# sidward14/gan-lab

Hardware: AMD Instinct MI355X
Metric: images/sec (G+D step), StyleGAN 1024^2 bs32/GPU (higher is better)
Workload: dtype f32; 1 GPU; StyleGAN res_samples=1024 FFHQ-shaped synthetic, bs=32/GPU fp32, nonsaturating + R1(lambda=10) + drift, stabilised phase, 1 D-iter + 1 G-iter; global_batch=32, per_gpu_batch=32, parallelism=single

## Files before the change

gan_lab_amd/csrc/pointwise.hip:

```cpp
#include "common.h"

#include <stdlib.h>

namespace {

constexpr int kMaxBlocks = 256 * 8;

inline unsigned ew_blocks(long long n_items) {
  long long b = (n_items + 255) / 256;
  if (b < 1) b = 1;
  if (b > kMaxBlocks) b = kMaxBlocks;
  return (unsigned)b;
}

struct ChunkRange { long long begin, end, stride; };
__device__ __forceinline__ ChunkRange chunk_range(long long hw4, int chunks, int c, int contig) {
  ChunkRange r;
  if (contig) {
    const long long rows = (hw4 + 255) / 256, per = (rows + chunks - 1) / chunks;
    r.begin = (long long)c * per * 256;
    r.end = r.begin + per * 256;
    if (r.end > hw4) r.end = hw4;
    r.stride = 256;
  } else {
// ... 298 lines not shown
  const double inv = 1.0 / (double)HW;
  const double k = rd * ys, a1 = (double)s1[pl] * inv, a2 = (double)s2[pl] * inv;
  const float* pg = gy + pl * HW;
  const float* px = x + pl * HW;
  const float* pn = (want_nw && noise) ? noise + (long long)n * HW : nullptr;
  float* po = out + pl * HW;
  const int lane = threadIdx.x & 63;
  double sb = 0.0, snw = 0.0;
  auto zval = [&](float g, float v) -> double {
    double t = k * ((double)g - a1 - ((double)v - md) * rd * a2);
    if (act == GANLAB_ACT_LRELU && !(v > 0.f)) t *= (double)slope;
    return t;
  };
  for (long long base = chunk * 256LL; base < per_n; base += (long long)chunks * 256) {
    const long long i = base + threadIdx.x;
    const bool live = i < per_n;
    const long long ii = live ? i : per_n - 1;
    const int rr = (int)(ii / w4), q = (int)(ii - (long long)rr * w4);
    const int y0 = R * rr, x0 = 4 * q;
    float h[R + 2][4];
#pragma unroll
    for (int kk = 0; kk < R + 2; ++kk) {
      const int yy = y0 - 1 + kk;
      const bool valid = (unsigned)yy < (unsigned)H;
      const long long ro = (long long)yy * W;
      float z[4] = {0.f, 0.f, 0.f, 0.f};
      if (valid) {
        float g[4], v[4];
        *reinterpret_cast<float4*>(g) = *reinterpret_cast<const float4*>(pg + ro + x0);
        *reinterpret_cast<float4*>(v) = *reinterpret_cast<const float4*>(px + ro + x0);
        const bool own = live && kk >= 1 && kk <= R;
        float nz[4] = {0.f, 0.f, 0.f, 0.f};
        if (own && pn) *reinterpret_cast<float4*>(nz) = *reinterpret_cast<const float4*>(pn + ro + x0);
#pragma unroll
        for (int j = 0; j < 4; ++j) {
          const double t = zval(g[j], v[j]);
          z[j] = (float)t;
          if (own) {
            sb += t;
            snw += t * (double)nz[j];
          }
        }
      }
      float l = __shfl_up(z[3], 1, 64);
      float r = __shfl_down(z[0], 1, 64);
      const bool need_l = lane == 0 && q != 0, need_r = lane == 63 && q != w4 - 1;
      float e = 0.f;
      if (valid && (need_l || need_r)) {
        const long long eo = ro + x0 + (need_l ? -1 : 4);
        e = (float)zval(pg[eo], px[eo]);
      }
      if (q == 0) l = 0.f;
      else if (lane == 0) l = e;
      if (q == w4 - 1) r = 0.f;
      else if (lane == 63) r = e;
      h[kk][0] = l + 2.f * z[0] + z[1];
      h[kk][1] = z[0] + 2.f * z[1] + z[2];
      h[kk][2] = z[1] + 2.f * z[2] + z[3];
      h[kk][3] = z[2] + 2.f * z[3] + r;
    }
    if (!live) continue;
#pragma unroll
    for (int kk = 0; kk < R; ++kk) {
      float4 o;
      o.x = (h[kk][0] + 2.f * h[kk + 1][0] + h[kk + 2][0]) * 0.0625f;
      o.y = (h[kk][1] + 2.f * h[kk + 1][1] + h[kk + 2][1]) * 0.0625f;
      o.z = (h[kk][2] + 2.f * h[kk + 1][2] + h[kk + 2][2]) * 0.0625f;
      o.w = (h[kk][3] + 2.f * h[kk + 1][3] + h[kk + 2][3]) * 0.0625f;
      *reinterpret_cast<float4*>(po + (long long)(y0 + kk) * W + x0) = o;
    }
  }
  const long long slot = ((long long)c * N + n) * chunks + chunk;
  if (want_b) {
    sb = gl_block_sum_256d(sb, red);
    if (threadIdx.x == 0) part[slot] = sb;
  }
  if (want_nw) {
    if (want_b) __syncthreads();
    snw = gl_block_sum_256d(snw, red);
    if (threadIdx.x == 0) part[(long long)C * N * chunks + slot] = snw;
  }
}

inline int blur_rows(int H) { return (H & 3) == 0 ? 4 : 2; }
inline int blur_rows_mode(int H, int mode) {
  const int min8 = mode == BF_FWD ? 512 : (mode == BF_A ? 256 : (1 << 30));
  return ((H & 7) == 0 && H >= min8) ? 8 : blur_rows(H);
}
#define BLUR_FUSED_LAUNCH(MODE, ...)                                                                   \
  do {                                                                                                 \
    const int rows_ = blur_rows_mode(H, MODE);                                                         \
    if (rows_ == 8) GL_LAUNCH((blur_fused_kernel<MODE, 8>), dim3(chunks, C), dim3(256), 0, ST, __VA_ARGS__);      \
    else if (rows_ == 4) GL_LAUNCH((blur_fused_kernel<MODE, 4>), dim3(chunks, C), dim3(256), 0, ST, __VA_ARGS__); \
    else GL_LAUNCH((blur_fused_kernel<MODE, 2>), dim3(chunks, C), dim3(256), 0, ST, __VA_ARGS__);                \
  } while (0)

#define BLUR_FUSED_LAUNCH_BITS(MODE, ...)                                                                            \
  do {                                                                                                               \
    const int rows_ = blur_rows_mode(H, MODE);                                                                       \
    if (rows_ == 8) GL_LAUNCH((blur_fused_kernel<MODE, 8, false, true>), dim3(chunks, C), dim3(256), 0, ST, __VA_ARGS__);      \
    else if (rows_ == 4) GL_LAUNCH((blur_fused_kernel<MODE, 4, false, true>), dim3(chunks, C), dim3(256), 0, ST, __VA_ARGS__); \
    else GL_LAUNCH((blur_fused_kernel<MODE, 2, false, true>), dim3(chunks, C), dim3(256), 0, ST, __VA_ARGS__);                \
  } while (0)

inline int blur_fused_chunks(int N, int H, int W) {
  long long c = ((long long)N * (H / blur_rows(H)) * (W / 4) + 256 * 4 - 1) / (256 * 4);
  if (c < 1) c = 1;
  if (c > 128) c = 128;
  return (int)c;
}

__global__ __launch_bounds__(256) void bias_act_stats_kernel(const float* __restrict__ x, const float* __restrict__ bias,
                                                             const float* __restrict__ noise,
                                                             const float* __restrict__ noise_w, float* __restrict__ y,
                                                             double* __restrict__ spart, int C, long long hw4,
                                                             int chunks, float bias_scale, int act, float slope,
                                                             int contig) {
  __shared__ double dred[2][4];
  const long long pl = blockIdx.y;
  const int c = (int)(pl % C);
  const long long n = pl / C;
  const float b = bias ? bias[c] * bias_scale : 0.f;
  const float nw = noise ? noise_w[c] : 0.f;
  const float4* xp = reinterpret_cast<const float4*>(x) + pl * hw4;
  const float4* np = noise ? reinterpret_cast<const float4*>(noise) + n * hw4 : nullptr;
  float4* yp = reinterpret_cast<float4*>(y) + pl * hw4;
  double ds = 0.0, dss = 0.0;
  const ChunkRange cr = chunk_range(hw4, chunks, blockIdx.x, contig);
  for (long long i = cr.begin + threadIdx.x; i < cr.end; i += cr.stride) {
    float v[4], nz[4] = {0.f, 0.f, 0.f, 0.f};
    *reinterpret_cast<float4*>(v) = xp[i];
    if (np) *reinterpret_cast<float4*>(nz) = np[i];
#pragma unroll
    for (int k = 0; k < 4; ++k) {
      float t = v[k] + b + nw * nz[k];
      if (act == GANLAB_ACT_LRELU) t = gl_lrelu(t, slope);
      v[k] = t;
      const double d = (double)t;
      ds += d;
      dss += d * d;
    }
    yp[i] = *reinterpret_cast<float4*>(v);
  }
#pragma unroll
  for (int o = 32; o > 0; o >>= 1) {
    ds += __shfl_xor(ds, o, 64);
    dss += __shfl_xor(dss, o, 64);
  }
  if ((threadIdx.x & 63) == 0) {
    dred[0][threadIdx.x >> 6] = ds;
    dred[1][threadIdx.x >> 6] = dss;
  }
  __syncthreads();
  if (threadIdx.x < 2) {
    const int k = threadIdx.x;
    spart[(pl * chunks + blockIdx.x) * 2 + k] = (dred[k][0] + dred[k][1]) + (dred[k][2] + dred[k][3]);
  }
}

__global__ void act_stats_finish_kernel(const double* __restrict__ spart, float* __restrict__ mean,
                                        float* __restrict__ rstd, long long planes, int chunks, double inv_hw, float eps) {
  const long long pl = blockIdx.x * (long long)blockDim.x + threadIdx.x;
  if (pl >= planes) return;
  double s = 0.0, ss = 0.0;
  for (int k = 0; k < chunks; ++k) {
    s += spart[(pl * chunks + k) * 2];
    ss += spart[(pl * chunks + k) * 2 + 1];
  }
  const double m = s * inv_hw;
  double var = ss * inv_hw - m * m;
  if (var < 0.0) var = 0.0;
  mean[pl] = (float)m;
  rstd[pl] = (float)(1.0 / sqrt(var + (double)eps));
}

__global__ __launch_bounds__(256) void row_stats_partial_kernel(const float* __restrict__ x, double* __restrict__ spart,
                                                                int chunks, long long m4) {
  __shared__ double red[2][4];
  const long long row = blockIdx.x / chunks;
  const int k = blockIdx.x % chunks;
  const long long per = (m4 + chunks - 1) / chunks, lo = k * per, hi = lo + per < m4 ? lo + per : m4;
  const float4* p4 = reinterpret_cast<const float4*>(x) + row * m4;
  double s = 0.0, ss = 0.0;
  for (long long i = lo + threadIdx.x; i < hi; i += 256) {
    const float4 v = p4[i];
    const double a = (double)v.x, b = (double)v.y, c = (double)v.z, d = (double)v.w;
    s += (a + b) + (c + d);
    ss += (a * a + b * b) + (c * c + d * d);
  }
#pragma unroll
  for (int o = 32; o > 0; o >>= 1) {
    s += __shfl_xor(s, o, 64);
    ss += __shfl_xor(ss, o, 64);
// ... 1158 lines not shown
  if (gb) GL_LAUNCH(channel_sum_stage2, dim3(C), dim3(64), 0, ST, (const double*)part, gb, C, N * chunks, bias_scale);
  if (gnw)
    GL_LAUNCH(channel_sum_stage2, dim3(C), dim3(64), 0, ST, (const double*)part + (size_t)C * N * chunks, gnw, C,
              N * chunks, 1.f);
  return GL_CHECK_LAUNCH();
}

int ganlab_instnorm_bwd_rgb_supported(int N, int C, int crgb, long long HW) {
  return (N > 0 && N <= 65535 && C > 0 && C <= 16 && crgb > 0 && crgb <= 4 && HW >= 1024 && (HW & 3) == 0) ? 1 : 0;
}

static RgbSrc make_rgb_src(const float* grgb, const float* wp, int crgb, int C) {
  RgbSrc r;
  r.grgb = grgb; r.wp = wp; r.crgb = crgb; r.cout_p = (C + 63) / 64 * 64;
  return r;
}

size_t ganlab_instnorm_bwd_reduce_rgb_workspace(int N, int C, long long HW) {
  if (!ganlab_instnorm_bwd_rgb_supported(N, C, 3, HW)) return 0;
  return (size_t)N * C * act_stats_chunks(HW / 4) * 2 * sizeof(double);
}

int ganlab_instnorm_style_bwd_reduce_rgb_f32(const float* grgb, const float* wp, int crgb, const float* x,
                                             const float* mean, const float* rstd, float* s1, float* s2, int N, int C,
                                             long long HW, void* workspace, size_t workspace_bytes, void* stream) {
  if (!grgb || !wp || !x || !mean || !rstd || !s1 || !s2) return GANLAB_EINVAL;
  if (!ganlab_instnorm_bwd_rgb_supported(N, C, crgb, HW)) return GANLAB_EUNSUPPORTED;
  if (!workspace || workspace_bytes < ganlab_instnorm_bwd_reduce_rgb_workspace(N, C, HW)) return GANLAB_EWORKSPACE;
  const long long hw4 = HW / 4, planes = (long long)N * C;
  const int chunks = act_stats_chunks(hw4);
  double* part = reinterpret_cast<double*>(workspace);
  if (C == RGB_MAXC && crgb == 3)
    GL_LAUNCH(instnorm_bwd_reduce_rgb_kernel<true>, dim3((unsigned)chunks, (unsigned)N), dim3(256), 0, ST,
              make_rgb_src(grgb, wp, crgb, C), x, mean, rstd, part, C, hw4, chunks, pw_contig());
  else
    GL_LAUNCH(instnorm_bwd_reduce_rgb_kernel<false>, dim3((unsigned)chunks, (unsigned)N), dim3(256), 0, ST,
              make_rgb_src(grgb, wp, crgb, C), x, mean, rstd, part, C, hw4, chunks, pw_contig());
  GL_LAUNCH(instnorm_bwd_reduce_rgb_finish_kernel, dim3((unsigned)((planes + 63) / 64)), dim3(64), 0, ST,
            (const double*)part, s1, s2, planes, chunks);
  return GL_CHECK_LAUNCH();
}

int ganlab_instnorm_style_bwd_act_rgb_f32(const float* grgb, const float* wp, int crgb, const float* x, const float* mean,
                                          const float* rstd, const float* style, const float* s1, const float* s2,
                                          const float* noise, float* gz, float* gb, float* gnw, int N, int C, long long HW,
                                          int act, float slope, float bias_scale, void* workspace, size_t workspace_bytes,
                                          void* stream) {
  if (!grgb || !wp || !x || !mean || !rstd || !s1 || !s2 || !gz || (gnw && !noise)) return GANLAB_EINVAL;
  if (!ganlab_instnorm_bwd_rgb_supported(N, C, crgb, HW)) return GANLAB_EUNSUPPORTED;
  if ((gb || gnw) && (!workspace || workspace_bytes < ganlab_instnorm_bwd_act_workspace(N, C, HW)))
    return GANLAB_EWORKSPACE;
  const long long hw4 = HW / 4;
  const int chunks = act_stats_chunks(hw4);
  double* part = reinterpret_cast<double*>(workspace);
  if (C == RGB_MAXC && crgb == 3 && act == GANLAB_ACT_LRELU)
    GL_LAUNCH(instnorm_bwd_apply_act_rgb_kernel<true>, dim3((unsigned)chunks, (unsigned)N), dim3(256), 0, ST,
              make_rgb_src(grgb, wp, crgb, C), x, mean, rstd, style, s1, s2, noise, gz, part, N, C, hw4, chunks, act, slope,
              gb ? 1 : 0, gnw ? 1 : 0, pw_contig());
  else
    GL_LAUNCH(instnorm_bwd_apply_act_rgb_kernel<false>, dim3((unsigned)chunks, (unsigned)N), dim3(256), 0, ST,
              make_rgb_src(grgb, wp, crgb, C), x, mean, rstd, style, s1, s2, noise, gz, part, N, C, hw4, chunks, act, slope,
              gb ? 1 : 0, gnw ? 1 : 0, pw_contig());
  if (gb) GL_LAUNCH(channel_sum_stage2, dim3(C), dim3(64), 0, ST, (const double*)part, gb, C, N * chunks, bias_scale);
  if (gnw)
    GL_LAUNCH(channel_sum_stage2, dim3(C), dim3(64), 0, ST, (const double*)part + (size_t)C * N * chunks, gnw, C,
              N * chunks, 1.f);
  return GL_CHECK_LAUNCH();
}

int ganlab_instnorm_style_bwd_act_blur_f32(const float* gy, const float* x, const float* mean, const float* rstd,
                                           const float* style, const float* s1, const float* s2, const float* noise,
                                           float* out, float* gb, float* gnw, int N, int C, int H, int W, int act,
                                           float slope, float bias_scale, void* workspace, size_t workspace_bytes,
                                           void* stream) {
  if (!gy || !x || !mean || !rstd || !s1 || !s2 || !out || N <= 0 || C <= 0 || (gnw && !noise)) return GANLAB_EINVAL;
  if (!ganlab_blur_fused_supported(H, W) || N > 65535 || C > 65535) return GANLAB_EUNSUPPORTED;
  const long long HW = (long long)H * W;
  if ((gb || gnw) && (!workspace || workspace_bytes < ganlab_instnorm_bwd_act_workspace(N, C, HW))) return GANLAB_EWORKSPACE;
  const int rows = blur_rows(H);
  const long long per_n = (long long)(H / rows) * (W / 4);
  int chunks = (int)((per_n + 256 * 4 - 1) / (256 * 4));
  if (chunks < 1) chunks = 1;
  if (chunks > 64) chunks = 64;
  double* part = reinterpret_cast<double*>(workspace);
  const dim3 grid((unsigned)chunks, (unsigned)C, (unsigned)N);
  if (rows == 4)
    GL_LAUNCH(instnorm_bwd_act_blur_kernel<4>, grid, dim3(256), 0, ST, gy, x, mean, rstd, style, s1, s2, noise, out, part, N, C,
              H, W, chunks, act, slope, gb ? 1 : 0, gnw ? 1 : 0);
  else
    GL_LAUNCH(instnorm_bwd_act_blur_kernel<2>, grid, dim3(256), 0, ST, gy, x, mean, rstd, style, s1, s2, noise, out, part, N, C,
              H, W, chunks, act, slope, gb ? 1 : 0, gnw ? 1 : 0);
  if (gb) GL_LAUNCH(channel_sum_stage2, dim3(C), dim3(64), 0, ST, (const double*)part, gb, C, N * chunks, bias_scale);
  if (gnw)
    GL_LAUNCH(channel_sum_stage2, dim3(C), dim3(64), 0, ST, (const double*)part + (size_t)C * N * chunks, gnw, C,
              N * chunks, 1.f);
  return GL_CHECK_LAUNCH();
}

int ganlab_bias_act_stats_f32(const float* x, const float* bias, const float* noise, const float* noise_w, float* y,
                              float* mean, float* rstd, int N, int C, long long HW, float bias_scale, int act,
                              float slope, float eps, void* workspace, size_t workspace_bytes, void* stream) {
  if (!x || !y || !mean || !rstd || N <= 0 || C <= 0 || HW <= 0 || (noise && !noise_w)) return GANLAB_EINVAL;
  if ((HW & 3) != 0) return GANLAB_EUNSUPPORTED;
  if (!workspace || workspace_bytes < ganlab_act_stats_workspace(N, C, HW)) return GANLAB_EWORKSPACE;
  const long long hw4 = HW / 4, planes = (long long)N * C;
  const int chunks = act_stats_chunks(hw4);
  double* sp = reinterpret_cast<double*>(workspace);
  GL_LAUNCH(bias_act_stats_kernel, dim3((unsigned)chunks, (unsigned)planes), dim3(256), 0, ST, x, bias, noise, noise_w,
            y, sp, C, hw4, chunks, bias_scale, act, slope, pw_contig());
  GL_LAUNCH(act_stats_finish_kernel, dim3((unsigned)((planes + 255) / 256)), dim3(256), 0, ST, (const double*)sp, mean,
            rstd, planes, chunks, 1.0 / (double)HW, eps);
  return GL_CHECK_LAUNCH();
}

int ganlab_blur_bias_act_stats_f32(const float* x, const float* bias, const float* noise, const float* noise_w,
                                   float* y, float* mean, float* rstd, int N, int C, int H, int W, float bias_scale,
                                   int act, float slope, float eps, void* workspace, size_t workspace_bytes,
                                   void* stream) {
  if (!x || !y || !mean || !rstd || N <= 0 || C <= 0 || (noise && !noise_w)) return GANLAB_EINVAL;
  if (!ganlab_blur_fused_supported(H, W)) return GANLAB_EUNSUPPORTED;
  if (!workspace || workspace_bytes < ganlab_act_stats_workspace(N, C, (long long)H * W)) return GANLAB_EWORKSPACE;
  const int rows = blur_rows_mode(H, BF_FWD);
  long long per_n = (long long)(H / rows) * (W / 4);
  int chunks = (int)((per_n + 256 * 4 - 1) / (256 * 4));
  if (chunks < 1) chunks = 1;
  if (chunks > 128) chunks = 128;
  double* sp = reinterpret_cast<double*>(workspace);
  const dim3 grid((unsigned)chunks, (unsigned)C, (unsigned)N);
  if (rows == 8)
    GL_LAUNCH((blur_fused_kernel<BF_FWD, 8, true>), grid, dim3(256), 0, ST, x, (const float*)nullptr, noise, bias,
              noise_w, y, (double*)nullptr, N, C, H, W, chunks, bias_scale, act, slope, 0, sp);
  else if (rows == 4)
    GL_LAUNCH((blur_fused_kernel<BF_FWD, 4, true>), grid, dim3(256), 0, ST, x, (const float*)nullptr, noise, bias,
              noise_w, y, (double*)nullptr, N, C, H, W, chunks, bias_scale, act, slope, 0, sp);
  else
    GL_LAUNCH((blur_fused_kernel<BF_FWD, 2, true>), grid, dim3(256), 0, ST, x, (const float*)nullptr, noise, bias,
              noise_w, y, (double*)nullptr, N, C, H, W, chunks, bias_scale, act, slope, 0, sp);
  const long long planes = (long long)N * C;
  GL_LAUNCH(act_stats_finish_kernel, dim3((unsigned)((planes + 255) / 256)), dim3(256), 0, ST, (const double*)sp, mean,
            rstd, planes, chunks, 1.0 / ((double)H * W), eps);
  return GL_CHECK_LAUNCH();
}

int ganlab_blur_act_bwd_f32(const float* g, const float* y, float* out, float* gb, int N, int C, int H, int W,
                            float slope, float bias_scale, void* workspace, size_t workspace_bytes, void* stream) {
  if (!g || !y || !out || N <= 0 || C <= 0) return GANLAB_EINVAL;
  if (!ganlab_blur_fused_supported(H, W)) return GANLAB_EUNSUPPORTED;
  const int chunks = blur_fused_chunks(N, H, W);
  if (gb && (!workspace || workspace_bytes < (size_t)C * chunks * sizeof(double))) return GANLAB_EWORKSPACE;
  BLUR_FUSED_LAUNCH(BF_A, g, y, (const float*)nullptr, (const float*)nullptr, (const float*)nullptr, out,
                    (double*)workspace, N, C, H, W, chunks, 1.f, 0, slope, gb ? 1 : 0);
  if (gb) GL_LAUNCH(channel_sum_stage2, dim3(C), dim3(64), 0, ST, (const double*)workspace, gb, C, chunks, bias_scale);
  return GL_CHECK_LAUNCH();
}

int ganlab_blur_act_bwd_bits_f32(const float* g, const unsigned* ybits, float* out, float* gb, int N, int C, int H, int W,
                                 float slope, float bias_scale, void* workspace, size_t workspace_bytes, void* stream) {
  if (!g || !ybits || !out || N <= 0 || C <= 0) return GANLAB_EINVAL;
  if (!ganlab_blur_fused_supported(H, W) || !ganlab_mask_bits_supported(H, W)) return GANLAB_EUNSUPPORTED;
  const int chunks = blur_fused_chunks(N, H, W);
  if (gb && (!workspace || workspace_bytes < (size_t)C * chunks * sizeof(double))) return GANLAB_EWORKSPACE;
  BLUR_FUSED_LAUNCH_BITS(BF_A, g, reinterpret_cast<const float*>(ybits), (const float*)nullptr, (const float*)nullptr,
                         (const float*)nullptr, out, (double*)workspace, N, C, H, W, chunks, 1.f, 0, slope, gb ? 1 : 0);
  if (gb) GL_LAUNCH(channel_sum_stage2, dim3(C), dim3(64), 0, ST, (const double*)workspace, gb, C, chunks, bias_scale);
  return GL_CHECK_LAUNCH();
}

int ganlab_act_bwd_blur_bits_f32(const float* g, const unsigned* ybits, const float* noise, float* out, float* gb,
                                 float* gnw, int N, int C, int H, int W, float slope, float bias_scale, void* workspace,
                                 size_t workspace_bytes, void* stream) {
  if (!g || !ybits || !out || N <= 0 || C <= 0 || (gnw && !noise)) return GANLAB_EINVAL;
  if (!ganlab_blur_fused_supported(H, W) || !ganlab_mask_bits_supported(H, W)) return GANLAB_EUNSUPPORTED;
  const int chunks = blur_fused_chunks(N, H, W);
  const int sums = (gb || gnw) ? 1 : 0;
  if (sums && (!workspace || workspace_bytes < (size_t)2 * C * chunks * sizeof(double))) return GANLAB_EWORKSPACE;
  BLUR_FUSED_LAUNCH_BITS(BF_AT, g, reinterpret_cast<const float*>(ybits), gnw ? noise : (const float*)nullptr,
                         (const float*)nullptr, (const float*)nullptr, out, (double*)workspace, N, C, H, W, chunks, 1.f, 0,
                         slope, sums);
  if (gb) GL_LAUNCH(channel_sum_stage2, dim3(C), dim3(64), 0, ST, (const double*)workspace, gb, C, chunks, bias_scale);
  if (gnw)
    GL_LAUNCH(channel_sum_stage2, dim3(C), dim3(64), 0, ST, (const double*)workspace + (size_t)C * chunks, gnw, C,
              chunks, 1.f);
  return GL_CHECK_LAUNCH();
}

int ganlab_act_bwd_blur_f32(const float* g, const float* y, const float* noise, float* out, float* gb, float* gnw,
                            int N, int C, int H, int W, float slope, float bias_scale, void* workspace,
                            size_t workspace_bytes, void* stream) {
  if (!g || !y || !out || N <= 0 || C <= 0 || (gnw && !noise)) return GANLAB_EINVAL;
  if (!ganlab_blur_fused_supported(H, W)) return GANLAB_EUNSUPPORTED;
  const int chunks = blur_fused_chunks(N, H, W);
  const int sums = (gb || gnw) ? 1 : 0;
  if (sums && (!workspace || workspace_bytes < (size_t)2 * C * chunks * sizeof(double))) return GANLAB_EWORKSPACE;
  BLUR_FUSED_LAUNCH(BF_AT, g, y, gnw ? noise : (const float*)nullptr, (const float*)nullptr, (const float*)nullptr, out,
                    (double*)workspace, N, C, H, W, chunks, 1.f, 0, slope, sums);
  if (gb) GL_LAUNCH(channel_sum_stage2, dim3(C), dim3(64), 0, ST, (const double*)workspace, gb, C, chunks, bias_scale);
  if (gnw)
    GL_LAUNCH(channel_sum_stage2, dim3(C), dim3(64), 0, ST, (const double*)workspace + (size_t)C * chunks, gnw, C,
              chunks, 1.f);
  return GL_CHECK_LAUNCH();
}

int ganlab_instnorm_stats_f32(const float* x, float* mean, float* rstd, long long planes, long long HW, float eps,
                              void* stream) {
  if (!x || !mean || !rstd || planes <= 0 || HW <= 0) return GANLAB_EINVAL;
  const int vec = ((HW & 3) == 0 && (reinterpret_cast<uintptr_t>(x) & 15) == 0) ? 1 : 0;
  if (HW >= 1024)
    GL_LAUNCH(instnorm_stats_kernel<256>, dim3((unsigned)planes), dim3(256), 0, ST, x, mean, rstd, planes,
                       HW, eps, vec);
  else
    GL_LAUNCH(instnorm_stats_kernel<64>, dim3((unsigned)((planes + 3) / 4)), dim3(256), 0, ST, x, mean,
                       rstd, planes, HW, eps, vec);
  return GL_CHECK_LAUNCH();
}

size_t ganlab_row_stats_workspace(long long rows, long long M) {
  if (rows <= 0 || M <= 0) return 0;
  return (size_t)rows * act_stats_chunks(M / 4) * 2 * sizeof(double);
}

int ganlab_row_stats_f32(const float* x, float* mean, float* rstd, long long rows, long long M, float eps,
                         void* workspace, size_t workspace_bytes, void* stream) {
  if (!x || !mean || !rstd || rows <= 0 || M <= 0) return GANLAB_EINVAL;
  const int chunks = act_stats_chunks(M / 4);
  if ((M & 3) != 0 || chunks < 2 || rows * chunks > 0x7fffffffLL || (reinterpret_cast<uintptr_t>(x) & 15) != 0)
    return ganlab_instnorm_stats_f32(x, mean, rstd, rows, M, eps, stream);
  if (!workspace || workspace_bytes < ganlab_row_stats_workspace(rows, M)) return GANLAB_EWORKSPACE;
  double* sp = reinterpret_cast<double*>(workspace);
  GL_LAUNCH(row_stats_partial_kernel, dim3((unsigned)(rows * chunks)), dim3(256), 0, ST, x, sp, chunks, M >> 2);
  GL_LAUNCH(act_stats_finish_kernel, dim3((unsigned)((rows + 255) / 256)), dim3(256), 0, ST, (const double*)sp, mean,
            rstd, rows, chunks, 1.0 / (double)M, eps);
  return GL_CHECK_LAUNCH();
}

int ganlab_instnorm_style_fwd_f32(const float* x, const float* mean, const float* rstd, const float* style,
                                  float* y, int N, int C, long long HW, void* stream) {
  if (!x || !mean || !rstd || !y || N <= 0 || C <= 0 || HW <= 0) return GANLAB_EINVAL;
  static const int chunk_u = [] {
    const char* e = getenv("GANLAB_PW_CHUNK");
    const int v = e ? atoi(e) : 2;
    return (v == 0 || v == 2 || v == 4 || v == 8) ? v : 2;
  }();
  if (chunk_u > 0 && HW % (1024 * 8) == 0 && (long long)N * C * (HW / (1024 * chunk_u)) < 0x7fffffffLL) {
    const int chunks = (int)(HW / (1024 * chunk_u));
    const unsigned grid = (unsigned)((long long)N * C * chunks);
    if (chunk_u == 8) GL_LAUNCH(instnorm_style_fwd_chunk_kernel<8>, dim3(grid), dim3(256), 0, ST, x, mean, rstd, style, y, C, chunks, HW);
    else if (chunk_u == 2) GL_LAUNCH(instnorm_style_fwd_chunk_kernel<2>, dim3(grid), dim3(256), 0, ST, x, mean, rstd, style, y, C, chunks, HW);
    else GL_LAUNCH(instnorm_style_fwd_chunk_kernel<4>, dim3(grid), dim3(256), 0, ST, x, mean, rstd, style, y, C, chunks, HW);
  } else if ((HW & 3) == 0)
    GL_LAUNCH(instnorm_style_fwd_kernel<4>, dim3(ew_blocks((long long)N * C * HW / 4)), dim3(256), 0, ST,
                       x, mean, rstd, style, y, N, C, HW);
  else
    GL_LAUNCH(instnorm_style_fwd_kernel<1>, dim3(ew_blocks((long long)N * C * HW)), dim3(256), 0, ST, x,
                       mean, rstd, style, y, N, C, HW);
  return GL_CHECK_LAUNCH();
}

int ganlab_instnorm_style_bwd_reduce_f32(const float* gy, const float* x, const float* mean, const float* rstd,
                                         float* s1, float* s2, long long planes, long long HW, void* stream) {
  if (!gy || !x || !mean || !rstd || !s1 || !s2 || planes <= 0 || HW <= 0) return GANLAB_EINVAL;
  if (HW >= 1024)
    GL_LAUNCH(instnorm_bwd_reduce_kernel<256>, dim3((unsigned)planes), dim3(256), 0, ST, gy, x, mean,
                       rstd, s1, s2, planes, HW);
  else
    GL_LAUNCH(instnorm_bwd_reduce_kernel<64>, dim3((unsigned)((planes + 3) / 4)), dim3(256), 0, ST, gy, x,
                       mean, rstd, s1, s2, planes, HW);
  return GL_CHECK_LAUNCH();
}

int ganlab_instnorm_style_bwd_apply_f32(const float* gy, const float* x, const float* mean, const float* rstd,
                                        const float* style, const float* s1, const float* s2, float* gx, int N,
                                        int C, long long HW, void* stream) {
  if (!gy || !x || !mean || !rstd || !s1 || !s2 || !gx || N <= 0 || C <= 0 || HW <= 0) return GANLAB_EINVAL;
  if ((HW & 3) == 0)
    GL_LAUNCH(instnorm_bwd_apply_kernel<4>, dim3(ew_blocks((long long)N * C * HW / 4)), dim3(256), 0, ST,
                       gy, x, mean, rstd, style, s1, s2, gx, N, C, HW);
  else
    GL_LAUNCH(instnorm_bwd_apply_kernel<1>, dim3(ew_blocks((long long)N * C * HW)), dim3(256), 0, ST, gy,
// ... 210 lines not shown
```

gan_lab_amd/ops.py:

```python
import ctypes
import os

import numpy as np

import torch
from torch.autograd import Function
from torch.autograd.function import once_differentiable

from . import _lib
from ._lib import ACT_LRELU, ACT_NONE, PACK_DGRAD, PACK_FWD, ConvGeom, check
from ._ops.core import (
    _p, _RAW_STREAM, _GET_DEVICE, _st, _c, _inplace, _same_numel, _gpu_device, _new, _ct, _aligned16, _nchw, _row_workspace,
    _INPUT_GRAD_ONLY, input_grad_only, _want_param_grads, _NO_GRAD_TOWARDS, no_grad_towards, _wants_input_grad, _DIRECT, _SINK,
    _TAKEN, _TAKE_HITS, direct_grads_enabled, direct_param_grads, _sink, _take, arena_takes, _sunk)
from ._ops.geom import (
    _COMPUTE, set_compute_dtype, get_compute_dtype, compute_dtype, Geom, pool_fusable, _OBSERVER, set_launch_observer, conv_flops,
    _note)
from ._ops.pointwise import (
    k_blur, decode_u8, k_up2, k_pool2, RESAMPLE_MODES, _RESAMPLE_TABLES, resample_matrix, _taps, _resample_tables, k_resample,
    k_bias_act, k_act_bwd, k_act_bwd_bias, k_channel_sum, k_axpby, k_scale_dev, k_sum, _ActBwd, _ActBwdBias, _ChanSum,
    _GroupBroadcast, _Blur, _Pool2, _Up2, _Resample, _Scale, _Axpby, _PixelNorm, _ChanAffine, _Mul, _Tanh, _TanhBwd, chan_affine,
    mul, tanh, channel_sum, blur, avg_pool2, upsample2, resample, lerp, scale, add, global_avg_pool, pixelnorm, group_broadcast)
from ._ops.norm import (
    _BatchNormTrain, batch_norm_composed, _ln_rowsums, _ln_project, _LayerNorm, _LayerNormBwd, layer_norm, layer_norm_composed)
# ... 549 lines not shown
    check(L.ganlab_conv_s2_fwd_blur_tail_f32(_p(a), _p(wp), _p(s_), _p(t_), _p(bias), _p(noise), _p(noise_w), _p(y), _p(mean),
                                             _p(rstd), g.ref(), bias_scale, act, slope, eps, ctypes.c_void_p(ws.data_ptr()),
                                             ws.numel() * 8, _st()), 'conv_s2_fwd_blur_tail')
    return y, mean, rstd


def k_conv_s2_dgrad_blur_act(gy, w, bits, g, scale, slope, bias_scale, want_gb):
    gy, w = _c(gy, 'conv grad_out'), _c(w, 'conv weight')
    assert g.pool and tuple(gy.shape) == g.out_shape and bits.numel() * 32 == g.N * g.Cin * g.Hin * g.Win
    _note('dgrad', g)
    L = _lib.lib()
    gz = _new(g.in_shape, gy)
    gb = _new((g.Cin,), gy) if want_gb else None
    ws = torch.empty((L.ganlab_conv_s2_blur_workspace(g.ref()) + 7) // 8, dtype=torch.float64, device=gy.device) \
        if want_gb else None
    wp = _packed(w, PACK_DGRAD, scale, s2_up=0)
    check(L.ganlab_conv_s2_dgrad_blur_act_bits_f32(_p(gy), _p(wp), bits.data_ptr(), _p(gz), _p(gb), g.ref(), slope, bias_scale,
                                                   ctypes.c_void_p(ws.data_ptr()) if ws is not None else None,
                                                   ws.numel() * 8 if ws is not None else 0, _st()),
          'conv_s2_dgrad_blur_act_bits')
    return gz, gb


def k_conv_wgrad(gy, x, g, scale):
    gy, x = _c(gy, 'conv grad_out'), _c(x, 'conv input')
    assert tuple(gy.shape) == g.out_shape and tuple(x.shape) == g.in_shape
    _note('wgrad', g)
    L = _lib.lib()
    gw = _take('gw', (g.Cout, g.Cin, g.ks, g.ks), x)
    if x3_wgrad_ok(g):
        return _wgrad_x3(gy, x, None, None, gw, g, scale)
    if g.bf is not None:
        if g.bf_fused is not None:
            nbytes = L.ganlab_conv_wgrad_bf16_workspace(ctypes.byref(g.bf_fused))
            if nbytes > 0:
                ws = torch.empty((nbytes + 3) // 4, dtype=torch.float32, device=x.device)
                check(L.ganlab_conv_wgrad_bf16(_p(gy), _p(x), _p(gw), ctypes.byref(g.bf_fused), scale, _p(ws),
                                               ws.numel() * 4, _st()), 'conv_wgrad_bf16')
                return gw
        xin = k_up2(x, 1.0) if g.up else x
        if g.pool:
            gy = k_up2(gy, 0.25)
        nbytes = L.ganlab_conv_wgrad_bf16_workspace(ctypes.byref(g.bf))
        if nbytes == 0:
            nbytes = L.ganlab_conv_wgrad_workspace(ctypes.byref(g.bf))
            ws = torch.empty((max(nbytes, 4) + 3) // 4, dtype=torch.float32, device=x.device)
            check(L.ganlab_conv_wgrad_f32(_p(gy), _p(xin), _p(gw), ctypes.byref(g.bf), scale, _p(ws), ws.numel() * 4,
                                          _st()), 'conv_wgrad')
            return gw
        ws = torch.empty((max(nbytes, 4) + 3) // 4, dtype=torch.float32, device=x.device)
        check(L.ganlab_conv_wgrad_bf16(_p(gy), _p(xin), _p(gw), ctypes.byref(g.bf), scale, _p(ws), ws.numel() * 4,
                                       _st()), 'conv_wgrad_bf16')
        return gw
    if g.s2:
        if x3_s2_wgrad_ok(g):
            return _wgrad_x3_s2(gy, x, None, None, gw, g, scale)
        nbytes = L.ganlab_conv_s2_wgrad_workspace(g.ref())
        ws = torch.empty((max(nbytes, 4) + 3) // 4, dtype=torch.float32, device=x.device)
        check(L.ganlab_conv_s2_wgrad_f32(_p(gy), _p(x), _p(gw), g.ref(), scale, _p(ws), ws.numel() * 4, _st()),
              'conv_s2_wgrad')
        return gw
    nbytes = L.ganlab_conv_wgrad_workspace(g.ref())
    ws = torch.empty((max(nbytes, 4) + 3) // 4, dtype=torch.float32, device=x.device)
    check(L.ganlab_conv_wgrad_f32(_p(gy), _p(x), _p(gw), g.ref(), scale, _p(ws), ws.numel() * 4, _st()),
          'conv_wgrad')
    return gw


_MASK_BITS = [None]


def mask_bits_ok(x):
    if _MASK_BITS[0] is None:
        import os
        _MASK_BITS[0] = os.environ.get('GANLAB_MASK_BITS') != '0'
    return _MASK_BITS[0] and x.dim() == 4 and bool(_lib.lib().ganlab_mask_bits_supported(int(x.shape[2]), int(x.shape[3])))


def mask_bits_ok_plane():
    if _MASK_BITS[0] is None:
        import os
        _MASK_BITS[0] = os.environ.get('GANLAB_MASK_BITS') != '0'
    return _MASK_BITS[0]


def k_blur_bits(x):
    x = _c(x)
    n, c, h, w = x.shape
    y = torch.empty_like(x)
    bits = torch.empty((x.numel() // 32,), dtype=torch.int32, device=x.device)
    check(_lib.lib().ganlab_blur3x3_bits_f32(_p(x), _p(y), bits.data_ptr(), n * c, h, w, _st()), 'blur3x3_bits')
    return y, bits


def _is_bits(y):
    return y.dtype == torch.int32


def blur_fusable(x):
    return x.dim() == 4 and bool(_lib.lib().ganlab_blur_fused_supported(int(x.shape[2]), int(x.shape[3])))


def _blur_ws(x):
    n, c, h, w = x.shape
    nbytes = _lib.lib().ganlab_blur_fused_workspace(n, c, h, w)
    return torch.empty((max(nbytes, 4) + 3) // 4, dtype=torch.float32, device=x.device)


def k_blur_bias_act(x, bias, noise, noise_w, bias_scale, act, slope):
    x = _c(x)
    n, c, h, w = x.shape
    bias = _c(bias) if bias is not None else None
    if noise is not None:
        noise, noise_w = _c(noise), _c(noise_w)
        assert noise.numel() == n * h * w and noise_w.numel() == c
    y = torch.empty_like(x)
    check(_lib.lib().ganlab_blur_bias_act_f32(_p(x), _p(bias), _p(noise), _p(noise_w), _p(y), n, c, h, w, bias_scale,
                                              act, slope, _st()), 'blur_bias_act')
    return y


def _stats_out(x, n, c, hw):
    L = _lib.lib()
    ws = torch.empty((max(L.ganlab_act_stats_workspace(n, c, hw), 8) + 7) // 8, dtype=torch.float64, device=x.device)
    return _new((n * c,), x), _new((n * c,), x), ws


def k_blur_bias_act_stats(x, bias, noise, noise_w, bias_scale, act, slope, eps):
    x = _c(x)
    n, c, h, w = x.shape
    bias = _c(bias) if bias is not None else None
    if noise is not None:
        noise, noise_w = _c(noise), _c(noise_w)
        assert noise.numel() == n * h * w and noise_w.numel() == c
    y = torch.empty_like(x)
    mean, rstd, ws = _stats_out(x, n, c, h * w)
    check(_lib.lib().ganlab_blur_bias_act_stats_f32(_p(x), _p(bias), _p(noise), _p(noise_w), _p(y), _p(mean), _p(rstd),
                                                    n, c, h, w, bias_scale, act, slope, eps, _p(ws), ws.numel() * 8,
                                                    _st()), 'blur_bias_act_stats')
    return y, mean, rstd


def k_bias_act_stats(x, bias, noise, noise_w, bias_scale, act, slope, eps):
    x = _c(x)
    n, c, hw = _nchw(x)
    y = torch.empty_like(x)
    bias = _c(bias) if bias is not None else None
    noise = _c(noise) if noise is not None else None
    noise_w = _c(noise_w) if noise_w is not None else None
    if noise is not None:
        assert noise.numel() == n * hw and noise_w.numel() == c
    mean, rstd, ws = _stats_out(x, n, c, hw)
    check(_lib.lib().ganlab_bias_act_stats_f32(_p(x), _p(bias), _p(noise), _p(noise_w), _p(y), _p(mean), _p(rstd), n, c,
                                               hw, bias_scale, act, slope, eps, _p(ws), ws.numel() * 8, _st()),
          'bias_act_stats')
    return y, mean, rstd


def k_blur_act_bwd(g, y, slope, bias_scale, want_gb):
    g = _c(g)
    n, c, h, w = g.shape
    out = torch.empty_like(g)
    gb = _take('gb', (c,), g) if want_gb else None
    ws = _blur_ws(g) if want_gb else None
    if _is_bits(y):
        assert y.numel() * 32 == g.numel()
# ... 1191 lines not shown
```

Before: 167.5 images/sec.

## Add rolling-row blur kernels that stream tall row strips with register reuse

Adds a rolling-row 3x3 blur walker where each thread owns a 4-wide column and walks a strip of up to 64 rows. It keeps two horizontally blurred rows in registers, so each input row is loaded once instead of being reloaded with halo overlap for every small row tile. The walker is used for the fused forward bias/noise/act/stats blur, the transposed act-backward blur (mask or bits) and the instnorm backward blur whenever the tensor is large enough. The trade-off is fewer parallel work items and longer serial per-thread loops. Cross-lane shuffles and edge loads handle the horizontal halo, and an env var can turn the path off.

```diff
diff --git a/gan_lab_amd/csrc/blur_roll.h b/gan_lab_amd/csrc/blur_roll.h
--- /dev/null
+++ b/gan_lab_amd/csrc/blur_roll.h
@@ -0,0 +1,267 @@
+#pragma once
+
+constexpr int kRollU = 4;
+
+inline int blur_roll_rows(long long planes, int H, int W) {
+  const char* e = getenv("GANLAB_BLUR_ROLL");
+  if (e && e[0] == '0') return 0;
+  if (H < 16 || (W & 3) != 0) return 0;
+  const int cand[3] = {64, 32, 16};
+  for (int S : cand) {
+    if (S > H) continue;
+    const long long items = planes * ((H + S - 1) / S) * (W >> 2);
+    if (items >= 16384LL * 64) return S;
+  }
+  return 0;
+}
+
+struct RollState { float h0[4], h1[4]; };
+
+template <int U, class Load, class Edge, class Emit>
+__device__ __forceinline__ void blur_roll_steps(RollState& st, int k0, int H, int y0, int rs, int q, int w4, bool live,
+                                                Load& load, Edge& edge, Emit& emit) {
+  const int lane = threadIdx.x & 63, x0 = 4 * q;
+  const bool need_l = lane == 0 && q != 0, need_r = lane == 63 && q != w4 - 1;
+  const int ylo = y0 > 0 ? y0 - 1 : 0, yhi = y0 + rs < H ? y0 + rs : H - 1;
+  float v[U][4], e[U];
+#pragma unroll
+  for (int u = 0; u < U; ++u) {
+    const int k = k0 + u, yy = y0 - 1 + k;
+    const bool valid = k <= rs + 1 && (unsigned)yy < (unsigned)H;
+    const int yc = yy < ylo ? ylo : (yy > yhi ? yhi : yy);
+    load(yc, live && k >= 1 && k <= rs, v[u]);
+    e[u] = 0.f;
+    if (need_l || need_r) e[u] = edge(yc, x0 + (need_l ? -1 : 4));
+    if (!valid) v[u][0] = v[u][1] = v[u][2] = v[u][3] = e[u] = 0.f;
+  }
+#pragma unroll
+  for (int u = 0; u < U; ++u) {
+    const int k = k0 + u, yy = y0 - 1 + k;
+    float l = __shfl_up(v[u][3], 1, 64);
+    float r = __shfl_down(v[u][0], 1, 64);
+    if (q == 0) l = 0.f;
+    else if (lane == 0) l = e[u];
+    if (q == w4 - 1) r = 0.f;
+    else if (lane == 63) r = e[u];
+    float h2[4];
+    h2[0] = l + 2.f * v[u][0] + v[u][1];
+    h2[1] = v[u][0] + 2.f * v[u][1] + v[u][2];
+    h2[2] = v[u][1] + 2.f * v[u][2] + v[u][3];
+    h2[3] = v[u][2] + 2.f * v[u][3] + r;
+    if (live && k >= 2 && k <= rs + 1) {
+      float o[4];
+#pragma unroll
+      for (int j = 0; j < 4; ++j) o[j] = (st.h0[j] + 2.f * st.h1[j] + h2[j]) * 0.0625f;
+      emit(yy - 1, o);
+    }
+#pragma unroll
+    for (int j = 0; j < 4; ++j) {
+      st.h0[j] = st.h1[j];
+      st.h1[j] = h2[j];
+    }
+  }
+}
+
+template <int U = kRollU, class Load, class Edge, class Emit>
+__device__ __forceinline__ void blur_roll_walk(int H, int S, int y0, int rs, int q, int w4, bool live, Load load, Edge edge,
+                                               Emit emit) {
+  RollState st;
+#pragma unroll
+  for (int j = 0; j < 4; ++j) st.h0[j] = st.h1[j] = 0.f;
+  blur_roll_steps<2>(st, 0, H, y0, rs, q, w4, live, load, edge, emit);
+  for (int k0 = 2; k0 < S + 2; k0 += U) blur_roll_steps<U>(st, k0, H, y0, rs, q, w4, live, load, edge, emit);
+}
+
+struct RollItem { long long pl; int y0, rs, q; };
+__device__ __forceinline__ RollItem roll_item(long long i, int H, int S, int ns, int w4) {
+  RollItem it;
+  it.q = (int)(i % w4);
+  const long long t = i / w4;
+  it.pl = t / ns;
+  it.y0 = (int)(t - it.pl * ns) * S;
+  it.rs = H - it.y0 < S ? H - it.y0 : S;
+  return it;
+}
+
+__device__ __forceinline__ void roll_ld4(float (&v)[4], const float* __restrict__ p) {
+  *reinterpret_cast<float4*>(v) = *reinterpret_cast<const float4*>(p);
+}
+
+template <int MODE, bool STATS = false, bool BITS = false>
+__global__ __launch_bounds__(256) void blur_roll_fused_kernel(const float* __restrict__ in, const float* __restrict__ y,
+                                                              const float* __restrict__ noise,
+                                                              const float* __restrict__ bias,
+                                                              const float* __restrict__ noise_w, float* __restrict__ out,
+                                                              double* __restrict__ part, int N, int C, int H, int W,
+                                                              int chunks, float bias_scale, int act, float slope,
+                                                              int want_sums, double* __restrict__ spart, int S) {
+  static_assert((MODE == BF_FWD && STATS && !BITS) || (MODE == BF_AT && !STATS), "forms on the rolling-row walker");
+  __shared__ double red[4];
+  __shared__ double dred[2][4];
+  const int c = blockIdx.y, chunk = blockIdx.x;
+  const int w4 = W >> 2, ns = (H + S - 1) / S;
+  const long long per_n = (long long)ns * w4, total = STATS ? per_n : (long long)N * per_n, HW = (long long)H * W;
+  const unsigned* __restrict__ yb = reinterpret_cast<const unsigned*>(y);
+  double ds = 0.0, dss = 0.0;
+  const float b = (MODE == BF_FWD && bias) ? bias[c] * bias_scale : 0.f;
+  const float nw = (MODE == BF_FWD && noise) ? noise_w[c] : 0.f;
+  double s0 = 0.0, s1 = 0.0;
+  for (long long base = chunk * 256LL; base < total; base += (long long)chunks * 256) {
+    const long long i = base + threadIdx.x;
+    const bool live = i < total;
+    const RollItem it = roll_item(live ? i : total - 1, H, S, ns, w4);
+    const long long n = STATS ? (long long)blockIdx.z : it.pl;
+    const long long plane = (n * C + c) * HW;
+    const float* pin = in + plane;
+    const float* pn = noise ? noise + n * HW : nullptr;
+    const int x0 = 4 * it.q;
+    blur_roll_walk(
+        H, S, it.y0, it.rs, it.q, w4, live,
+        [&](int yy, bool own, float(&v)[4]) {
+          const long long ro = (long long)yy * W + x0;
+          roll_ld4(v, pin + ro);
+          if constexpr (MODE == BF_AT) {
+            if constexpr (BITS) {
+              const unsigned nb = mask_nibble(yb, plane + ro);
+#pragma unroll
+              for (int j = 0; j < 4; ++j) v[j] = ((nb >> j) & 1u) ? v[j] : v[j] * slope;
+            } else {
+              float m[4];
+              roll_ld4(m, y + plane + ro);
+#pragma unroll
+              for (int j = 0; j < 4; ++j) v[j] = m[j] > 0.f ? v[j] : v[j] * slope;
+            }
+            if (own) {
+              float nz[4] = {0.f, 0.f, 0.f, 0.f};
+              if (pn && want_sums) roll_ld4(nz, pn + ro);
+#pragma unroll
+              for (int j = 0; j < 4; ++j) {
+                s0 += (double)v[j];
+                s1 += (double)v[j] * nz[j];
+              }
+            }
+          }
+        },
+        [&](int yy, int xe) {
+          const long long eo = (long long)yy * W + xe;
+          float e = pin[eo];
+          if constexpr (MODE == BF_AT) {
+            if constexpr (BITS) e = mask_bit(yb, plane + eo) ? e : e * slope;
+            else e = y[plane + eo] > 0.f ? e : e * slope;
+          }
+          return e;
+        },
+        [&](int yy, float(&o)[4]) {
+          const long long ro = (long long)yy * W + x0;
+          if constexpr (MODE == BF_FWD) {
+            float nz[4] = {0.f, 0.f, 0.f, 0.f};
+            if (pn) roll_ld4(nz, pn + ro);
+#pragma unroll
+            for (int j = 0; j < 4; ++j) {
+              float t = o[j] + b + nw * nz[j];
+              if (act == GANLAB_ACT_LRELU) t = gl_lrelu(t, slope);
+              o[j] = t;
+              if (STATS) {
+                const double d = (double)t;
+                ds += d;
+                dss += d * d;
+              }
+            }
+          }
+          *reinterpret_cast<float4*>(out + plane + ro) = *reinterpret_cast<float4*>(o);
+        });
+  }
+  if (STATS) {
+#pragma unroll
+    for (int o = 32; o > 0; o >>= 1) {
+      ds += __shfl_xor(ds, o, 64);
+      dss += __shfl_xor(dss, o, 64);
+    }
+    if ((threadIdx.x & 63) == 0) {
+      dred[0][threadIdx.x >> 6] = ds;
+      dred[1][threadIdx.x >> 6] = dss;
+    }
+    __syncthreads();
+    if (threadIdx.x < 2) {
+      const int k = threadIdx.x;
+      spart[(((long long)blockIdx.z * C + c) * chunks + chunk) * 2 + k] = (dred[k][0] + dred[k][1]) + (dred[k][2] + dred[k][3]);
+    }
+  }
+  if (MODE != BF_FWD && want_sums) {
+    s0 = gl_block_sum_256d(s0, red);
+    if (threadIdx.x == 0) part[(long long)c * chunks + chunk] = s0;
+    if (MODE == BF_AT) {
+      __syncthreads();
+      s1 = gl_block_sum_256d(s1, red);
+      if (threadIdx.x == 0) part[((long long)C + c) * chunks + chunk] = s1;
+    }
+  }
+}
+
+__global__ __launch_bounds__(256) void instnorm_bwd_act_blur_roll_kernel(
+    const float* __restrict__ gy, const float* __restrict__ x, const float* __restrict__ mean,
+    const float* __restrict__ rstd, const float* __restrict__ style, const float* __restrict__ s1,
+    const float* __restrict__ s2, const float* __restrict__ noise, float* __restrict__ out, double* __restrict__ part,
+    int N, int C, int H, int W, int chunks, int act, float slope, int want_b, int want_nw, int S) {
+  __shared__ double red[4];
+  const int c = blockIdx.y, n = blockIdx.z, chunk = blockIdx.x;
+  const long long pl = (long long)n * C + c, HW = (long long)H * W;
+  const int w4 = W >> 2, ns = (H + S - 1) / S;
+  const long long per_n = (long long)ns * w4;
+  const double md = (double)mean[pl], rd = (double)rstd[pl];
+  const double ys = style ? (double)style[((long long)n * 2 + 0) * C + c] + 1.0 : 1.0;
+  const double inv = 1.0 / (double)HW;
+  const double k = rd * ys, a1 = (double)s1[pl] * inv, a2 = (double)s2[pl] * inv;
+  const float* pg = gy + pl * HW;
+  const float* px = x + pl * HW;
+  const float* pn = (want_nw && noise) ? noise + (long long)n * HW : nullptr;
+  float* po = out + pl * HW;
+  double sb = 0.0, snw = 0.0;
+  auto zval = [&](float g, float v) -> double {
+    double t = k * ((double)g - a1 - ((double)v - md) * rd * a2);
+    if (act == GANLAB_ACT_LRELU && !(v > 0.f)) t *= (double)slope;
+    return t;
+  };
+  for (long long base = chunk * 256LL; base < per_n; base += (long long)chunks * 256) {
+    const long long i = base + threadIdx.x;
+    const bool live = i < per_n;
+    const RollItem it = roll_item(live ? i : per_n - 1, H, S, ns, w4);
+    const int x0 = 4 * it.q;
+    blur_roll_walk<2>(
+        H, S, it.y0, it.rs, it.q, w4, live,
+        [&](int yy, bool own, float(&z)[4]) {
+          const long long ro = (long long)yy * W + x0;
+          float g[4], v[4];
+          roll_ld4(g, pg + ro);
+          roll_ld4(v, px + ro);
+          float nz[4] = {0.f, 0.f, 0.f, 0.f};
+          if (own && pn) roll_ld4(nz, pn + ro);
+#pragma unroll
+          for (int j = 0; j < 4; ++j) {
+            const double t = zval(g[j], v[j]);
+            z[j] = (float)t;
+            if (own) {
+              sb += t;
+              snw += t * (double)nz[j];
+            }
+          }
+        },
+        [&](int yy, int xe) {
+          const long long eo = (long long)yy * W + xe;
+          return (float)zval(pg[eo], px[eo]);
+        },
+        [&](int yy, float(&o)[4]) {
+          *reinterpret_cast<float4*>(po + (long long)yy * W + x0) = *reinterpret_cast<float4*>(o);
+        });
+  }
+  const long long slot = ((long long)c * N + n) * chunks + chunk;
+  if (want_b) {
+    sb = gl_block_sum_256d(sb, red);
+    if (threadIdx.x == 0) part[slot] = sb;
+  }
+  if (want_nw) {
+    if (want_b) __syncthreads();
+    snw = gl_block_sum_256d(snw, red);
+    if (threadIdx.x == 0) part[(long long)C * N * chunks + slot] = snw;
+  }
+}
diff --git a/gan_lab_amd/csrc/pointwise.hip b/gan_lab_amd/csrc/pointwise.hip
--- a/gan_lab_amd/csrc/pointwise.hip
+++ b/gan_lab_amd/csrc/pointwise.hip
@@ -404,6 +404,8 @@
   }
 }
 
+#include "blur_roll.h"
+
 inline int blur_rows(int H) { return (H & 3) == 0 ? 4 : 2; }
 inline int blur_rows_mode(int H, int mode) {
   const int min8 = mode == BF_FWD ? 512 : (mode == BF_A ? 256 : (1 << 30));
@@ -431,6 +433,14 @@
   if (c > 128) c = 128;
   return (int)c;
 }
+
+inline int blur_roll_chunks(long long items, int cap) {
+  long long c = (items + 255) / 256;
+  if (c < 1) c = 1;
+  if (c > cap) c = cap;
+  return (int)c;
+}
+inline long long blur_roll_items(long long planes, int H, int W, int S) { return planes * ((H + S - 1) / S) * (W >> 2); }
 
 __global__ __launch_bounds__(256) void bias_act_stats_kernel(const float* __restrict__ x, const float* __restrict__ bias,
                                                              const float* __restrict__ noise,
@@ -1755,9 +1765,14 @@
   int chunks = (int)((per_n + 256 * 4 - 1) / (256 * 4));
   if (chunks < 1) chunks = 1;
   if (chunks > 64) chunks = 64;
+  const int S = blur_roll_rows((long long)N * C, H, W);
+  if (S) chunks = blur_roll_chunks(blur_roll_items(1, H, W, S), 64);
   double* part = reinterpret_cast<double*>(workspace);
   const dim3 grid((unsigned)chunks, (unsigned)C, (unsigned)N);
-  if (rows == 4)
+  if (S)
+    GL_LAUNCH(instnorm_bwd_act_blur_roll_kernel, grid, dim3(256), 0, ST, gy, x, mean, rstd, style, s1, s2, noise, out, part, N,
+              C, H, W, chunks, act, slope, gb ? 1 : 0, gnw ? 1 : 0, S);
+  else if (rows == 4)
     GL_LAUNCH(instnorm_bwd_act_blur_kernel<4>, grid, dim3(256), 0, ST, gy, x, mean, rstd, style, s1, s2, noise, out, part, N, C,
               H, W, chunks, act, slope, gb ? 1 : 0, gnw ? 1 : 0);
   else
@@ -1798,9 +1813,14 @@
   int chunks = (int)((per_n + 256 * 4 - 1) / (256 * 4));
   if (chunks < 1) chunks = 1;
   if (chunks > 128) chunks = 128;
+  const int S = blur_roll_rows((long long)N * C, H, W);
+  if (S) chunks = blur_roll_chunks(blur_roll_items(1, H, W, S), 128);
   double* sp = reinterpret_cast<double*>(workspace);
   const dim3 grid((unsigned)chunks, (unsigned)C, (unsigned)N);
-  if (rows == 8)
+  if (S)
+    GL_LAUNCH((blur_roll_fused_kernel<BF_FWD, true>), grid, dim3(256), 0, ST, x, (const float*)nullptr, noise, bias, noise_w, y,
+              (double*)nullptr, N, C, H, W, chunks, bias_scale, act, slope, 0, sp, S);
+  else if (rows == 8)
     GL_LAUNCH((blur_fused_kernel<BF_FWD, 8, true>), grid, dim3(256), 0, ST, x, (const float*)nullptr, noise, bias,
               noise_w, y, (double*)nullptr, N, C, H, W, chunks, bias_scale, act, slope, 0, sp);
   else if (rows == 4)
@@ -1847,9 +1867,14 @@
   const int chunks = blur_fused_chunks(N, H, W);
   const int sums = (gb || gnw) ? 1 : 0;
   if (sums && (!workspace || workspace_bytes < (size_t)2 * C * chunks * sizeof(double))) return GANLAB_EWORKSPACE;
-  BLUR_FUSED_LAUNCH_BITS(BF_AT, g, reinterpret_cast<const float*>(ybits), gnw ? noise : (const float*)nullptr,
-                         (const float*)nullptr, (const float*)nullptr, out, (double*)workspace, N, C, H, W, chunks, 1.f, 0,
-                         slope, sums);
+  if (const int S = blur_roll_rows((long long)N * C, H, W))
+    GL_LAUNCH((blur_roll_fused_kernel<BF_AT, false, true>), dim3(chunks, C), dim3(256), 0, ST, g,
+              reinterpret_cast<const float*>(ybits), gnw ? noise : (const float*)nullptr, (const float*)nullptr,
+              (const float*)nullptr, out, (double*)workspace, N, C, H, W, chunks, 1.f, 0, slope, sums, (double*)nullptr, S);
+  else
+    BLUR_FUSED_LAUNCH_BITS(BF_AT, g, reinterpret_cast<const float*>(ybits), gnw ? noise : (const float*)nullptr,
+                           (const float*)nullptr, (const float*)nullptr, out, (double*)workspace, N, C, H, W, chunks, 1.f, 0,
+                           slope, sums);
   if (gb) GL_LAUNCH(channel_sum_stage2, dim3(C), dim3(64), 0, ST, (const double*)workspace, gb, C, chunks, bias_scale);
   if (gnw)
     GL_LAUNCH(channel_sum_stage2, dim3(C), dim3(64), 0, ST, (const double*)workspace + (size_t)C * chunks, gnw, C,
@@ -1865,8 +1890,13 @@
   const int chunks = blur_fused_chunks(N, H, W);
   const int sums = (gb || gnw) ? 1 : 0;
   if (sums && (!workspace || workspace_bytes < (size_t)2 * C * chunks * sizeof(double))) return GANLAB_EWORKSPACE;
-  BLUR_FUSED_LAUNCH(BF_AT, g, y, gnw ? noise : (const float*)nullptr, (const float*)nullptr, (const float*)nullptr, out,
-                    (double*)workspace, N, C, H, W, chunks, 1.f, 0, slope, sums);
+  if (const int S = blur_roll_rows((long long)N * C, H, W))
+    GL_LAUNCH((blur_roll_fused_kernel<BF_AT>), dim3(chunks, C), dim3(256), 0, ST, g, y, gnw ? noise : (const float*)nullptr,
+              (const float*)nullptr, (const float*)nullptr, out, (double*)workspace, N, C, H, W, chunks, 1.f, 0, slope, sums,
+              (double*)nullptr, S);
+  else
+    BLUR_FUSED_LAUNCH(BF_AT, g, y, gnw ? noise : (const float*)nullptr, (const float*)nullptr, (const float*)nullptr, out,
+                      (double*)workspace, N, C, H, W, chunks, 1.f, 0, slope, sums);
   if (gb) GL_LAUNCH(channel_sum_stage2, dim3(C), dim3(64), 0, ST, (const double*)workspace, gb, C, chunks, bias_scale);
   if (gnw)
     GL_LAUNCH(channel_sum_stage2, dim3(C), dim3(64), 0, ST, (const double*)workspace + (size_t)C * chunks, gnw, C,
diff --git a/gan_lab_amd/ops.py b/gan_lab_amd/ops.py
--- a/gan_lab_amd/ops.py
+++ b/gan_lab_amd/ops.py
@@ -655,6 +655,12 @@
         import os
         _MASK_BITS[0] = os.environ.get('GANLAB_MASK_BITS') != '0'
     return _MASK_BITS[0]
+
+
+def set_blur_roll(enabled):
+    old = os.environ.get('GANLAB_BLUR_ROLL') != '0'
+    os.environ['GANLAB_BLUR_ROLL'] = '1' if enabled else '0'
+    return old
 
 
 def k_blur_bits(x):
```

Result: no change. 167.9 images/sec, median of 3 (+0.2%).
